# httpsworldview/openmeters

Measured on AMD Instinct MI355X. Metric: STFT frames/s (4096-pt Hann, hop 256, reassignment on), higher is better.
Workload: dtype f32

## Files before the change

openmeters_amd/csrc/buffer_device.hpp:

```cpp
#pragma once
#include <hip/hip_runtime.h>

#include "fft_device.hpp"

namespace omx {

struct GlobalBuffer {
    __amdgpu_buffer_rsrc_t rsrc;
};
__device__ __forceinline__ GlobalBuffer global_buffer(const void* base, uint32_t bytes) {
#ifdef OMX_BUFFER_NO_PIN
    return GlobalBuffer{__builtin_amdgcn_make_buffer_rsrc(const_cast<void*>(base), 0, (int)bytes, 0x00020000)};
#endif
    const uint64_t p = reinterpret_cast<uint64_t>(base);
    const uint32_t lo = (uint32_t)__builtin_amdgcn_readfirstlane((int)(uint32_t)p), hi = (uint32_t)__builtin_amdgcn_readfirstlane((int)(uint32_t)(p >> 32));
    const void* ub = reinterpret_cast<const void*>(((uint64_t)hi << 32) | lo);
    return GlobalBuffer{__builtin_amdgcn_make_buffer_rsrc(const_cast<void*>(ub), 0, __builtin_amdgcn_readfirstlane((int)bytes), 0x00020000)};
}
__device__ __forceinline__ float load_f32(const GlobalBuffer& b, uint32_t lane_bytes, uint32_t uniform_bytes) {
    return __builtin_bit_cast(float, __builtin_amdgcn_raw_buffer_load_b32(b.rsrc, (int)lane_bytes, (int)uniform_bytes, 0));
}
__device__ __forceinline__ v2f load_v2f(const GlobalBuffer& b, uint32_t lane_bytes, uint32_t uniform_bytes) {
    typedef unsigned u2 __attribute__((ext_vector_type(2)));
    const u2 u = __builtin_amdgcn_raw_buffer_load_b64(b.rsrc, (int)lane_bytes, (int)uniform_bytes, 0);
    return __builtin_bit_cast(v2f, u);
}

}
```

openmeters_amd/csrc/capi.cpp:

```cpp
#include "common.hpp"
#include "spectrogram.hpp"
#include "spectrum.hpp"
#include "loudness.hpp"
#include "stereometer.hpp"
#include "capture_group.hpp"
#include "oscilloscope.hpp"
#include "waveform.hpp"

namespace omx {
const std::string& last_error();
}
using namespace omx;

#define REQUIRE_DEVICE()                       \
    do {                                       \
        const int _rc = device_ready();        \
        if (_rc != OMX_NONE) return _rc;       \
    } while (0)

struct omx_spectrogram {
    SpectrogramSingle impl;
    explicit omx_spectrogram(const omx_spectrogram_config& c) : impl(c) {}
};
struct omx_spectrogram_bank {
// ... 228 lines not shown
    k_weighting_transition_debug(sample_rate, frames, out);
    return OMX_NONE;
}
int omx_debug_k2_phase_cycles(uint64_t* out, uint32_t n, int reset) {
    if (!out || n < (uint32_t)K2_PHASES) return OMX_ERR_INVALID;
    REQUIRE_DEVICE();
#ifndef OMX_TUNING
    (void)reset;
    set_last_error("omx_debug_k2_phase_cycles: phase-timing kernels exist only in the tuning build (make TUNING=1)");
    return OMX_ERR_UNSUPPORTED;
#else
    return guarded([&] {
        unsigned long long c[K2_PHASES];
        k2_phase_cycles(c, reset != 0);
        for (int i = 0; i < K2_PHASES; ++i) out[i] = c[i];
        return (int)K2_PHASES;
    });
#endif
}
int omx_spectrogram_bank_process_ragged(omx_spectrogram_bank* b, const float* pcm, uint64_t frames_capacity, const uint32_t* frames,
                                        const uint8_t* reset_mask, uint32_t channels, float sample_rate,
                                        const uint8_t positions[OMX_MAX_CHANNELS], void* stream, omx_spectrogram_ragged_update* out) {
    if (!b || !pcm || !frames || !positions) return OMX_ERR_INVALID;
    return guarded([&] {
        return b->impl.process_ragged(pcm, frames_capacity, frames, reset_mask, channels, sample_rate, positions, static_cast<hipStream_t>(stream), out);
    });
}
int omx_spectrogram_bank_set_option(omx_spectrogram_bank* b, uint32_t option, uint64_t value) {
    if (!b) return OMX_ERR_INVALID;
    switch (option) {
        case OMX_OPT_KERNEL_TIMING: b->impl.timer().enabled = value != 0; return OMX_NONE;
        case OMX_OPT_FORCE_GENERIC: b->impl.force_generic(value != 0); return OMX_NONE;
        case OMX_OPT_KERNEL_FORM:
            if (value != 0 && value != 1 && value != 2 && value != 30 && value != 31) return OMX_ERR_INVALID;
#ifndef OMX_TUNING
            if (value == 1 || value == 2) {
                set_last_error("OMX_OPT_KERNEL_FORM 1 / 2: superseded kernels, built by `make TUNING=1` (libomx_hip_tuning.so) only");
                return OMX_ERR_UNSUPPORTED;
            }
#endif
            b->impl.kernel_form((int)value);
            return OMX_NONE;
        default: return OMX_ERR_INVALID;
    }
}

void omx_spectrum_config_default(omx_spectrum_config* out) {
    if (out) spectrum_config_default(out);
}
int omx_spectrum_create(const omx_spectrum_config* cfg, omx_spectrum** out) {
    if (!cfg || !out) return OMX_ERR_INVALID;
    REQUIRE_DEVICE();
    return guarded([&] {
        *out = new omx_spectrum(*cfg);
        return (int)OMX_NONE;
    });
}
void omx_spectrum_destroy(omx_spectrum* h) { delete h; }
int omx_spectrum_get_config(const omx_spectrum* h, omx_spectrum_config* out) {
    if (!h || !out) return OMX_ERR_INVALID;
    *out = h->impl.bank.config();
    return OMX_NONE;
}
int omx_spectrum_update_config(omx_spectrum* h, const omx_spectrum_config* cfg) {
    if (!h || !cfg) return OMX_ERR_INVALID;
    return guarded([&] {
        h->impl.bank.update_config(*cfg, nullptr);
        return (int)OMX_NONE;
    });
}
// ... 632 lines not shown
```

openmeters_amd/csrc/spectrogram.cpp:

```cpp
#include "spectrogram.hpp"

namespace omx {

constexpr size_t kDefaultFftSize = 2048;
constexpr size_t kDefaultHopSize = 64;
constexpr size_t kMaxHistoryColumns = 8192;
constexpr size_t kHistoryByteBudget = 128u * 1024u * 1024u;

void spectrogram_config_default(omx_spectrogram_config* c) {
    std::memset(c, 0, sizeof(*c));
    c->sample_rate = kDefaultSampleRate;
    c->window = OMX_WINDOW_HANN;
    c->fft_size = kDefaultFftSize;
    c->hop_size = kDefaultHopSize;
    c->history_length = 0;
    c->zero_padding_factor = 1;
    c->use_reassignment = 1;
}

static void normalize(omx_spectrogram_config& c) {
    c.sample_rate = sanitize_sample_rate(c.sample_rate);
    if (c.fft_size == 0) c.fft_size = kDefaultFftSize;
    if (c.hop_size == 0) c.hop_size = std::max<uint64_t>(std::min<uint64_t>(kDefaultHopSize, c.fft_size), 1);
    c.zero_padding_factor = std::max<uint64_t>(c.zero_padding_factor, 1);
// ... 121 lines not shown
            OMX_HIP(hipStreamSynchronize(stream));
        }
        std::vector<float> tw(W);
        const float center = (float)(W ? W - 1 : 0) * 0.5f;
        for (size_t i = 0; i < W; ++i) tw[i] = ((float)i - center) * window[i];
        d_twindow_.upload(tw, stream);
        double sum = 0.0, squares = 0.0;
        for (float xf : window) {
            const double x = (double)xf;
            sum = sum + x;
            squares = squares + x * x;
        }
        power_scale_ = (float)(sum * sum / ((double)fft_size_ * squares));
    } else {
        power_scale_ = 1.0f;
    }
    fast4096_ = (W == fft_size_ && (W == 16384 || W == 8192 || W == 4096 || W == 2048 || W == 1024));
    const bool fast_classic_zp = !reassign && W < fft_size_ && W >= 256 &&
                                 (fft_size_ == 1024 || fft_size_ == 2048 || fft_size_ == 4096 || fft_size_ == 8192 || fft_size_ == 16384);
    fast_zp_ = reassign && W < fft_size_ &&
               (((W == 1024 || W == 2048 || W == 4096) && (fft_size_ == 2048 || fft_size_ == 4096 || fft_size_ == 8192)) ||
                ((W == 1024 || W == 2048 || W == 4096 || W == 8192) && fft_size_ == 16384));
    const bool residue_shape = W < fft_size_ && fft_size_ > 16384 && fft_size_ <= (size_t(1) << 19) && (fft_size_ & (fft_size_ - 1)) == 0 &&
                               (W == 1024 || W == 2048 || W == 4096 || W == 8192 || W == 16384);
    fast_zpr_ = reassign && residue_shape;
    classic_zpr_ = !reassign && residue_shape;
    if (fast_zpr_ || classic_zpr_) fast_zp_ = true;
    if (fast_classic_zp) {
        fast4096_ = true;
        d_tw256_.upload(twiddle_table(256, 256), stream);
        d_tw4096_.upload(twiddle_table(fft_size_, fft_size_), stream);
    } else if (fast4096_ || fast_zp_) {
        d_tw256_.upload(twiddle_table(256, 256), stream);
        d_tw4096_.upload(twiddle_table(W, W), stream);
        std::vector<float> half_tw = twiddle_table(2 * W, W);
        for (float& x : half_tw) x *= 0.5f;
        d_tw8192_.upload(half_tw, stream);
        if (fast_zp_) d_twF_.upload(twiddle_table(fft_size_, fft_size_), stream);
    }
    d_bin_norm_.upload(bin_norm, stream);
    OMX_HIP(hipStreamSynchronize(stream));
    prepared_ = true;

    const uint64_t buffered_len = (uint64_t)active_len * 2;
    const uint64_t pending = head_ - tail_;
    drain(pending > buffered_len ? pending - buffered_len : 0);
    pending_skip_ = 0;
}

void SpectrogramBank::prepare(hipStream_t stream) {
    if (!prepared_) rebuild_fft(stream);
}

void SpectrogramBank::update_config(const omx_spectrogram_config& in, hipStream_t stream) {
    omx_spectrogram_config cfg = in;
    normalize(cfg);
    const omx_spectrogram_config prev = cfg_;
    const bool prepared = prepared_;
    if (prepared) require_supported(cfg);
    const uint64_t old_read_len = prev.use_reassignment ? hilbert_len_ : prev.fft_size;
    cfg_ = cfg;
    const bool rate_changed = prev.sample_rate != cfg.sample_rate;
    const bool rebuild = prev.fft_size != cfg.fft_size || prev.zero_padding_factor != cfg.zero_padding_factor ||
                         prev.window != cfg.window || prev.use_reassignment != cfg.use_reassignment || rate_changed;
    if (rebuild && prepared) {
        rebuild_fft(stream);
        if (rate_changed) {
// ... 28 lines not shown
    if (cols) OMX_HIP(hipMemsetAsync(d_counts_.ptr, 0, (size_t)(n_streams_ * n_cols) * sizeof(uint32_t), stream));
    if (reassign) d_points_.reserve((size_t)(n_streams_ * n_cols * stride), pinned);
    else d_codes_.reserve((size_t)(n_streams_ * n_cols * stride), pinned);

    const float sr = cfg_.sample_rate;
    const float bin_hz = sr / (float)fft_size_;
    const float max_hz = sr * 0.5f;
    const float inv_2pi = sr / kTau;
    const float inv_hop = 1.0f / (float)hop;
    const float latency_hops = (float)center_offset * inv_hop;

    timer_.begin(stream);
    const bool fast = (fast4096_ || fast_zp_) && !force_generic_ && ring_cap_ <= (uint64_t(1) << 30) && hop <= 0xFFFFFFFFull;
    if (fast) {
        StftFastArgs fa{};
        fa.ring = ring_.ptr;
        fa.cap = ring_cap_;
        fa.tail = tail;
        fa.tails = tails;
        fa.cols = cols;
        fa.hop = (uint32_t)hop;
        fa.n_streams = n_streams_;
        fa.n_cols = (uint32_t)n_cols;
        fa.column_stride = (uint32_t)stride;
        fa.window_size = (uint32_t)W;
        fa.last_nonzero = last_nonzero_.ptr;
        fa.window = d_window_.ptr;
        fa.dwindow = d_dwindow_.ptr;
        fa.twindow = d_twindow_.ptr;
        fa.bin_norm = d_bin_norm_.ptr;
        fa.tw256 = reinterpret_cast<const v2f*>(d_tw256_.ptr);
        fa.tw4096 = reinterpret_cast<const v2f*>(d_tw4096_.ptr);
        fa.tw8192 = reinterpret_cast<const v2f*>(d_tw8192_.ptr);
        fa.bin_hz = bin_hz;
        fa.max_hz = max_hz;
        fa.inv_2pi = inv_2pi;
        fa.inv_hop = inv_hop;
        fa.latency_hops = latency_hops;
        fa.win_terms = (cfg_.window == OMX_WINDOW_HANN || cfg_.window == OMX_WINDOW_HAMMING) ? 2u : 0u;
        fa.win_c0 = cfg_.window == OMX_WINDOW_HANN ? 0.5f : 25.0f / 46.0f;
        fa.win_c1 = cfg_.window == OMX_WINDOW_HANN ? -0.5f : -21.0f / 46.0f;
        {
            static const float kCos[5][4] = {{1.0f, 0.0f, 0.0f, 0.0f},
                                             {0.5f, -0.5f, 0.0f, 0.0f},
                                             {25.0f / 46.0f, -21.0f / 46.0f, 0.0f, 0.0f},
                                             {0.42f, -0.5f, 0.08f, 0.0f},
                                             {0.35875f, -0.48829f, 0.14128f, -0.01168f}};
            static const uint32_t kTerms[5] = {1, 2, 2, 3, 4};
            const uint32_t wk = cfg_.window <= OMX_WINDOW_BLACKMAN_HARRIS ? cfg_.window : OMX_WINDOW_HANN;
            for (int m = 0; m < 4; ++m) fa.cos_c[m] = kCos[wk][m];
            fa.cos_terms = kTerms[wk];
        }
        fa.points = d_points_.ptr;
        fa.counts = d_counts_.ptr;
        if (!reassign) {
            d_col_sums_.reserve((size_t)(n_streams_ * n_cols));
            fa.col_sums = d_col_sums_.ptr;
        }
        const bool cross_check = kernel_form_ == 30;
        const bool split_check = kernel_form_ == 31;
        if (reassign && fft_size_ == 4096 && !fast_zp_ && split_check) {
            const uint64_t total = (uint64_t)n_streams_ * n_cols, chunk = std::min<uint64_t>(total, 4096);
            d_workspace_.reserve((size_t)(chunk * stft_big_scratch_bytes_per_frame() / sizeof(float)));
            for (uint64_t first = 0; first < total; first += chunk)
                launch_stft_reassigned_4096_split(fa, d_workspace_.ptr, (uint32_t)first, (uint32_t)std::min(chunk, total - first), stream);
        } else if (reassign && fft_size_ == 16384 && !fast_zp_) {
            const uint64_t total = (uint64_t)n_streams_ * n_cols, chunk = std::min<uint64_t>(total, 1024);
            d_workspace_.reserve((size_t)(chunk * stft_big_scratch_bytes_per_frame() / sizeof(float)));
            for (uint64_t first = 0; first < total; first += chunk)
                launch_stft_reassigned_16384(fa, d_workspace_.ptr, (uint32_t)first, (uint32_t)std::min(chunk, total - first), stream);
        } else if (fast_zpr_) {
            const uint64_t total = (uint64_t)n_streams_ * n_cols, per = stft_residue_scratch_bytes_per_frame((uint32_t)W, (uint32_t)fft_size_);
            const uint64_t chunk = std::min<uint64_t>(total, std::max<uint64_t>((uint64_t(512) << 20) / per, 1));
            d_workspace_.reserve((size_t)(chunk * per / sizeof(float)));
            for (uint64_t first = 0; first < total; first += chunk)
                (void)launch_stft_reassigned_residue(fa, (uint32_t)W, (uint32_t)(fft_size_ / W), reinterpret_cast<const v2f*>(d_twF_.ptr), d_workspace_.ptr,
                                                     (uint32_t)first, (uint32_t)std::min(chunk, total - first), stream);
        } else if (classic_zpr_) {
            (void)launch_stft_classic_residue(fa, d_codes_.ptr, (uint32_t)W, (uint32_t)(fft_size_ / W), reinterpret_cast<const v2f*>(d_twF_.ptr), stream);
        } else if (fast_zp_ && fft_size_ == 16384) {
            const uint64_t total = (uint64_t)n_streams_ * n_cols, chunk = std::min<uint64_t>(total, 1024);
            d_workspace_.reserve((size_t)(chunk * stft_big_scratch_bytes_per_frame() / sizeof(float)));
            for (uint64_t first = 0; first < total; first += chunk)
                (void)launch_stft_reassigned_zp_16384(fa, (uint32_t)W, reinterpret_cast<const v2f*>(d_twF_.ptr), d_workspace_.ptr,
                                                      (uint32_t)first, (uint32_t)std::min(chunk, total - first), stream);
        } else if (fast_zp_)
            (void)launch_stft_reassigned_zp(fa, (uint32_t)W, (uint32_t)fft_size_, reinterpret_cast<const v2f*>(d_twF_.ptr), stream);
// ... 390 lines not shown
```

openmeters_amd/csrc/spectrogram.hpp:

```cpp
#pragma once
#include "stft_kernels.hpp"

namespace omx {

void spectrogram_config_default(omx_spectrogram_config* c);
uint64_t col_byte_stride(uint32_t kind, uint32_t points);
uint64_t history_columns(uint32_t kind, uint32_t points, uint64_t requested);
uint16_t pack_classic_db_host(float db);

class SpectrogramBank {
public:
    SpectrogramBank(const omx_spectrogram_config& cfg, uint32_t n_streams);
    const omx_spectrogram_config& config() const { return cfg_; }
    void update_config(const omx_spectrogram_config& cfg, hipStream_t stream);
    void reset_audio();
    void prepare(hipStream_t stream);
    int process(const float* pcm, bool pcm_on_device, uint64_t frames, uint32_t channels, float sample_rate,
                const uint8_t positions[OMX_MAX_CHANNELS], hipStream_t stream, omx_spectrogram_bank_update* out);
    int push_begin(uint64_t frames, uint32_t channels, float sample_rate, hipStream_t stream, IngestSlots& slots);
    void push_end(const IngestSlots& slots);
    int process_pushed(hipStream_t stream, omx_spectrogram_bank_update* out);
    int process_ragged(const float* d_pcm, uint64_t frames_capacity, const uint32_t* frames, const uint8_t* reset_mask, uint32_t channels,
                       float sample_rate, const uint8_t positions[OMX_MAX_CHANNELS], hipStream_t stream, omx_spectrogram_ragged_update* out);
    int ragged_plan(const float* d_pcm, uint64_t frames_capacity, const uint32_t* frames, const uint8_t* reset_mask, uint32_t channels,
                    float sample_rate, const uint8_t positions[OMX_MAX_CHANNELS], hipStream_t stream, IngestArgs& ia_out);
    int ragged_finish(hipStream_t stream, omx_spectrogram_ragged_update* out);
    int fetch_column(uint64_t stream_index, uint64_t column, void* dst, uint64_t cap, uint64_t* n_out, hipStream_t stream);
    EventTimer& timer() { return timer_; }
    void force_generic(bool on) { force_generic_ = on; }
    void kernel_form(int form) { kernel_form_ = form; }
    void host_outputs(size_t limit_bytes) { host_output_limit_ = limit_bytes; }
    bool outputs_on_host() const { return d_counts_.pinned; }
    hipStream_t last_stream() const { return last_stream_; }

private:
    void rebuild_fft(hipStream_t stream);
    void launch_columns(uint64_t n_cols, uint64_t tail, const uint64_t* tails, const uint32_t* cols, hipStream_t stream);
    void enter_ragged(hipStream_t stream);
    void ensure_ring(uint64_t incoming, hipStream_t stream);
    void drain(uint64_t count);
    void advance(uint64_t count);
    void clear_last_nonzero(hipStream_t stream);

    omx_spectrogram_config cfg_{};
    uint32_t n_streams_;
    int kernel_form_ = 0;
    bool prepared_ = false, reset_ = true, fast4096_ = false, fast_zp_ = false, fast_zpr_ = false, classic_zpr_ = false, force_generic_ = false;
    size_t fft_size_ = 0, hilbert_len_ = 0;
    float power_scale_ = 1.0f;
    uint64_t head_ = 0, tail_ = 0, pending_skip_ = 0, ring_cap_ = 0;
    DeviceBuffer<float> ring_;
    HostStage staging_;
    DeviceBuffer<long long> last_nonzero_, partial_nonzero_;
    DeviceBuffer<float> d_window_, d_dwindow_, d_twindow_, d_bin_norm_, d_col_sums_;
    DeviceBuffer<float> d_tw_fft_, d_tw_hilbert_, d_tw256_, d_tw4096_, d_tw8192_, d_twF_, d_workspace_;
    DeviceBuffer<float> d_blu_chirp_, d_blu_bf_, d_blu_tw_;
    size_t blu_m_ = 0;
    OutBuffer<omx_spectrogram_point> d_points_;
    OutBuffer<uint32_t> d_counts_;
    OutBuffer<uint16_t> d_codes_;
    size_t host_output_limit_ = 0;
    uint64_t pend_max_cols_ = 0;
    bool ragged_ = false;
    uint64_t ragged_pending_bound_ = 0;
    DeviceBuffer<uint64_t> r_head_, r_tail_, r_skip_, r_ing_head_, r_col_tail_;
    DeviceBuffer<uint32_t> r_reset_flag_, r_ing_skip_, r_ing_count_, r_ncols_, r_reset_out_;
    DeviceView<uint32_t> r_frames_;
    DeviceView<uint8_t> r_mask_;
    RaggedStaging r_staging_;
    uint64_t last_cols_ = 0, last_stride_ = 0;
    uint32_t last_kind_ = OMX_COLUMN_REASSIGNED;
    EventTimer timer_;
    hipStream_t last_stream_ = nullptr;
};

struct SpectrogramSingle {
    SpectrogramBank bank;
    std::vector<uint64_t> offsets;
    std::vector<omx_spectrogram_point> points;
    std::vector<uint16_t> codes;
    explicit SpectrogramSingle(const omx_spectrogram_config& c) : bank(c, 1) { bank.host_outputs(size_t(2) << 20); }
    int process_block(const omx_block* block, omx_spectrogram_update* out);
};

}
```

openmeters_amd/csrc/stft4096_tri_kernels.hip:

```cpp
#include "stft_kernels.hpp"

#include <mutex>

#include "buffer_device.hpp"
#include "fft_device.hpp"
#include "fft_fused_device.hpp"
#include "reassign_device.hpp"
#include "twiddle_run_device.hpp"

namespace omx {

namespace {

#if !defined(TRI_KNOCK) || !defined(OMX_TUNING)
#undef TRI_KNOCK
#define TRI_KNOCK 0
#endif
#ifndef TRI_LDS_SYNC
#define TRI_LDS_SYNC 1
#endif
#if TRI_KNOCK == 3
#define TRI_SYNC() __builtin_amdgcn_sched_barrier(0)
#elif TRI_LDS_SYNC
#define TRI_SYNC() asm volatile("s_waitcnt lgkmcnt(0)\n\ts_barrier" ::: "memory")
#else
#define TRI_SYNC() __syncthreads()
#endif

__device__ __forceinline__ bool tri_block_to_stream_chunk(uint32_t n_streams, uint32_t chunks, uint32_t& s, uint32_t& chunk) {
    const uint32_t b = blockIdx.x;
    const uint32_t xcd = b & 7u, q = b >> 3;
    s = (q / chunks) * 8u + xcd;
    chunk = q % chunks;
    return s < n_streams;
}

template <int TT>
__device__ __forceinline__ v2f w8_at(v2f base) {
    return rotate128<4 * TT>(base);
}

#ifndef TRI_SWZ
#define TRI_SWZ 0
#endif
#if TRI_SWZ
constexpr int kTriSlots = 4096;
__device__ __forceinline__ int xslot(int j) { return j ^ ((j >> 4) & 15); }
__device__ __forceinline__ int per_call(int x) {
    asm volatile("" : "+v"(x));
// ... 88 lines not shown
#pragma unroll
    for (int t = 1; t < 16; ++t) w[t] = tw2[k * (unsigned)t];
    w[0] = w[1];
    dft16_fused_tw<INV>(v, w);
#else
#pragma unroll
    for (int t = 1; t < 16; ++t) v[t] = twmul<INV>(v[t], tw2[k * (unsigned)t]);
    dft16<INV>(v);
#endif
}
template <bool INV>
__device__ __forceinline__ void pass3_16(v2f (&v)[16], const v2f (&tw3)[15]) {
    if (TRI_KNOCK == 2) return;
#if TRI_FUSED
    v2f w[16];
#pragma unroll
    for (int t = 1; t < 16; ++t) w[t] = tw3[t - 1];
    w[0] = w[1];
    dft16_fused_tw<INV>(v, w);
#else
#pragma unroll
    for (int t = 1; t < 16; ++t) v[t] = twmul<INV>(v[t], tw3[t - 1]);
    dft16<INV>(v);
#endif
}
__device__ __forceinline__ void natural(v2f (&v)[16]) {
    v2f r[16];
#pragma unroll
    for (int t = 0; t < 16; ++t) r[t] = v[DFT16_OUT(t)];
#pragma unroll
    for (int t = 0; t < 16; ++t) v[t] = r[t];
}

template <bool INV>
__device__ __forceinline__ void tri_dual(v2f (&a)[16], v2f (&b)[16], v2f* X, const v2f* tw2, const v2f (&tw3)[15], int j) {
    plain16<INV>(a);
    x_write1(a, X, j);
    TRI_SYNC();
    x_read2(a, X, j);
    plain16<INV>(b);
    TRI_SYNC();
    x_write1(b, X, j);
    pass2_16<INV>(a, tw2, j);
    TRI_SYNC();
    x_read2(b, X, j);
    TRI_SYNC();
    x_write2(a, X, j);
    pass2_16<INV>(b, tw2, j);
    TRI_SYNC();
    x_read(a, X, j);
    TRI_SYNC();
    x_write2(b, X, j);
    pass3_16<INV>(a, tw3);
    natural(a);
    TRI_SYNC();
    x_read(b, X, j);
    pass3_16<INV>(b, tw3);
    natural(b);
}

__device__ __forceinline__ void store_point(omx_spectrogram_point* out, uint32_t pos, const omx_spectrogram_point& p) {
    *reinterpret_cast<omx_spectrogram_point*>(reinterpret_cast<char*>(out) + __umul24(pos, 12u)) = p;
}

}

constexpr size_t kTriLds = (size_t)kTriSlots * sizeof(v2f) + 4096 * sizeof(float) + 256 * sizeof(v2f) + 36 * sizeof(uint32_t) + 4 * sizeof(float);

template <int TERMS>
__global__ __launch_bounds__(256, 3) void stft_reassigned_4096_tri_kernel(StftFastArgs a) {
    extern __shared__ __attribute__((aligned(16))) unsigned char smem_raw[];
    v2f* X = reinterpret_cast<v2f*>(smem_raw);
    float* imb = reinterpret_cast<float*>(X + kTriSlots);
    v2f* tw2_lds = reinterpret_cast<v2f*>(imb + 4096);
    uint32_t* scan = reinterpret_cast<uint32_t*>(tw2_lds + 256);
    float* hil = reinterpret_cast<float*>(scan + 36);

    const uint32_t chunks = (a.n_cols + 1u) / 2u;
    uint32_t s, chunk;
    if (!tri_block_to_stream_chunk(a.n_streams, chunks, s, chunk)) return;
    const int j = threadIdx.x;
    const unsigned ju = threadIdx.x;
    const int lane = j & 63, wave = j >> 6;
    const int wave_u = __builtin_amdgcn_readfirstlane(wave);
    const float* ring = a.ring + (uint64_t)s * a.cap;
    const uint32_t mask32 = (uint32_t)(a.cap - 1);
    const uint32_t bytemask = mask32 << 2;
    const char* ring_bytes = reinterpret_cast<const char*>(ring);
    const long long last_nonzero = a.last_nonzero[s];
    const uint32_t* cols_p = a.cols;
    const uint64_t* tails_p = a.tails;
    const uint32_t n_cols_s = cols_p ? cols_p[s] : a.n_cols;
    const uint64_t tail_s = tails_p ? tails_p[s] : a.tail;
    const ReassignConsts rc{a.bin_hz, a.max_hz, a.inv_2pi, a.inv_hop, a.latency_hops};

    const uint32_t col0 = chunk * 2u;
    if (col0 >= n_cols_s) return;
    const bool have1 = col0 + 1u < n_cols_s;
    const uint32_t col1 = have1 ? col0 + 1u : col0;
    const uint64_t p0a = tail_s + (uint64_t)col0 * a.hop, p0b = tail_s + (uint64_t)col1 * a.hop;
    uint32_t* count_a = a.counts + (uint64_t)s * a.n_cols + col0;
    uint32_t* count_b = a.counts + (uint64_t)s * a.n_cols + col1;

    const uint32_t pa32 = (uint32_t)p0a, pb32 = (uint32_t)p0b;
    const uint32_t off_a = pa32 & mask32, hop_bytes = (pb32 - pa32) * 4u;
    const bool direct = (uint64_t)off_a + (uint64_t)(pb32 - pa32) + 8192ull <= a.cap && ((p0a | p0b) & 1ull) == 0;
    const GlobalBuffer windowb = global_buffer(ring + off_a, hop_bytes + 8192u * 4u);
    const GlobalBuffer tw4096b = global_buffer(a.tw4096, 4096u * 8u), tw8192b = global_buffer(a.tw8192, 4096u * 8u),
                       normb = global_buffer(a.bin_norm, 2049u * 4u), twinb = global_buffer(a.twindow, 4096u * 4u);

    v2f va[16], vb[16];
    if (TRI_KNOCK == 7) {
#pragma unroll
        for (int t = 0; t < 16; ++t) {
            va[t] = v2f{(float)(j + t) * 1e-4f, (float)(j - t) * 1e-4f};
            vb[t] = v2f{(float)(j + 2 * t) * 1e-4f, (float)(j - 3 * t) * 1e-4f};
        }
    } else if (direct) {
#pragma unroll
        for (int t = 0; t < 16; ++t) {
            va[t] = load_v2f(windowb, ju * 8u, 2048u * (unsigned)t);
            vb[t] = load_v2f(windowb, ju * 8u, hop_bytes + 2048u * (unsigned)t);
        }
    } else {
#pragma unroll
        for (int t = 0; t < 16; ++t) {
            const uint32_t qa = pa32 + 2u * (ju + 256u * (unsigned)t), qb = pb32 + 2u * (ju + 256u * (unsigned)t);
            va[t] = v2f{ring[qa & mask32], ring[(qa + 1u) & mask32]};
            vb[t] = v2f{ring[qb & mask32], ring[(qb + 1u) & mask32]};
        }
    }
    v2f tw3[15];
#pragma unroll
    for (int t = 1; t < 16; ++t) tw3[t - 1] = load_v2f(tw4096b, ju * 8u * (unsigned)t, 0);
    tw2_lds[j] = a.tw256[ju];
    const v2f w8_base = load_v2f(tw8192b, ju * 8u, 0);
    const bool silent_a = last_nonzero < (long long)p0a, silent_b = last_nonzero < (long long)p0b;
    if (silent_a && (silent_b || !have1)) {
        if (j == 0) {
            *count_a = 0;
            if (have1) *count_b = 0;
        }
        return;
    }
    tri_dual<false>(va, vb, X, tw2_lds, tw3, j);

    const int part = j ? xslot(256 - j) : kTriStep;
    auto hilbert_spectrum = [&](v2f (&y)[16], const v2f (&v)[16]) {
#pragma unroll
        for (int t = 0; t < 16; ++t) {
            const v2f z = v[t], zr = TRI_KNOCK == 8 ? v[15 - t] : X[part + kTriStep * (15 - t)];
            const v2f sum{z.x + zr.x, z.y - zr.y}, dif{z.x - zr.x, z.y + zr.y};
            v2f w8;
            switch (t) {
                case 0: w8 = w8_at<0>(w8_base); break;
                case 1: w8 = w8_at<1>(w8_base); break;
                case 2: w8 = w8_at<2>(w8_base); break;
                case 3: w8 = w8_at<3>(w8_base); break;
                case 4: w8 = w8_at<4>(w8_base); break;
                case 5: w8 = w8_at<5>(w8_base); break;
                case 6: w8 = w8_at<6>(w8_base); break;
                case 7: w8 = w8_at<7>(w8_base); break;
                case 8: w8 = w8_at<8>(w8_base); break;
                case 9: w8 = w8_at<9>(w8_base); break;
                case 10: w8 = w8_at<10>(w8_base); break;
                case 11: w8 = w8_at<11>(w8_base); break;
                case 12: w8 = w8_at<12>(w8_base); break;
                case 13: w8 = w8_at<13>(w8_base); break;
                case 14: w8 = w8_at<14>(w8_base); break;
                default: w8 = w8_at<15>(w8_base); break;
            }
            y[t] = TRI_KNOCK == 5 ? sum + dif : cmulc(sum, w8) - cmul(dif, w8);
            if (t == 0 && j == 0) y[t] = v2f{0.0f, 0.0f};
        }
    };
    v2f ya[16], yb[16];
    TRI_SYNC();
#pragma unroll
    for (int t = 0; t < 16; ++t) X[xslot(j) + kTriStep * t] = va[t];
    if (j == 0) {
        hil[0] = (va[0].x + va[0].y) * 0.5f;
// ... 22 lines not shown
            for (int t = 0; t < 16; ++t) xr[t] = *reinterpret_cast<const float*>(ring_bytes + (((q + 256u * (unsigned)t) << 2) & bytemask));
        }
    };
    auto load_twindow = [&](float (&twin)[16]) {
#pragma unroll
        for (int t = 0; t < 16; ++t) twin[t] = load_f32(twinb, ju * 4u, 1024u * (unsigned)t);
    };
    float xra[16], twina[16];
    load_real_half(xra, 0u, pa32);
    load_twindow(twina);
    TRI_SYNC();
    float* imag_a = reinterpret_cast<float*>(X);
#pragma unroll
    for (int t = 4; t < 12; ++t) {
        *reinterpret_cast<v2f*>(imag_a + 2 * (j + 256 * t - 1024)) = ya[t];
        *reinterpret_cast<v2f*>(imb + 2 * (j + 256 * t - 1024)) = yb[t];
    }
    TRI_SYNC();
    constexpr int REACH = TERMS > 1 ? TERMS - 1 : 1;
    const float c0 = a.cos_c[0];
    float half_c[REACH], dscale[REACH];
#pragma unroll
    for (int m = 1; m <= REACH; ++m) {
        half_c[m - 1] = TERMS > 1 ? 0.5f * a.cos_c[m] : 0.0f;
        dscale[m - 1] = TERMS > 1 ? a.cos_c[m] * ((float)m * 3.14159265358979323846f / 4096.0f) : 0.0f;
    }
    v2f* lin_z = X;

    struct ColumnPoints {
        omx_spectrogram_point pts[9];
        unsigned long long masks[9];
        uint32_t exc, running;
    };
    auto build = [&](v2f (&z)[16], v2f (&z2)[16], const float (&xr)[16], const float (&twin)[16], const float* imag, float half_x0, float half_xn) {
        const float par = (j & 1) ? -half_xn : half_xn;
#pragma unroll
        for (int t = 0; t < 16; ++t) {
            z[t] = v2f{4096.0f * xr[t] - half_x0 + par, imag[j + 256 * t]};
            z2[t] = v2f{z[t].x * twin[t], z[t].y * twin[t]};
        }
    };
    auto analyse = [&](v2f (&z)[16], v2f (&z2)[16], bool silent, ColumnPoints& o) {
        omx_spectrogram_point (&pts)[9] = o.pts;
        unsigned long long (&masks)[9] = o.masks;
        TRI_SYNC();
        tri_dual<false>(z, z2, X, tw2_lds, tw3, j);
        float pn[9];
#pragma unroll
        for (int t = 0; t < 9; ++t) pn[t] = load_f32(normb, ju * 4u, 1024u * (unsigned)t);
        TRI_SYNC();
#pragma unroll
        for (int t = 0; t < 8; ++t) lin_z[3 + j + 256 * t] = z[t];
        if (wave_u == 0) lin_z[3 + j + 2048] = z[8];
        if (j >= 253) lin_z[j - 253] = z[15];
        TRI_SYNC();
        auto bins = [&](auto first, auto last) {
            constexpr int T0 = decltype(first)::value, T1 = decltype(last)::value;
            v2f nzm[T1 - T0][REACH], nzp[T1 - T0][REACH];
            if constexpr (TERMS > 1) {
#pragma unroll
                for (int t = T0; t < T1; ++t)
#pragma unroll
                    for (int m = 1; m <= REACH; ++m) {
                        nzm[t - T0][m - 1] = lin_z[3 + j + 256 * t - m];
                        nzp[t - T0][m - 1] = lin_z[3 + j + 256 * t + m];
                    }
            }
#pragma unroll
            for (int t = T0; t < T1; ++t) {
                const uint32_t bin = (uint32_t)(j + 256 * t);
                v2f bb{c0 * z[t].x, c0 * z[t].y}, bd{0.0f, 0.0f};
// ... 33 lines not shown
            bins(std::integral_constant<int, 2>{}, std::integral_constant<int, 3>{});
            bins(std::integral_constant<int, 3>{}, std::integral_constant<int, 4>{});
            bins(std::integral_constant<int, 4>{}, std::integral_constant<int, 5>{});
            bins(std::integral_constant<int, 5>{}, std::integral_constant<int, 6>{});
            bins(std::integral_constant<int, 6>{}, std::integral_constant<int, 7>{});
            bins(std::integral_constant<int, 7>{}, std::integral_constant<int, 8>{});
        }
        if (wave_u == 0) {
            bins(std::integral_constant<int, 8>{}, std::integral_constant<int, 9>{});
        } else {
            masks[8] = 0ull;
            if (lane == 0) scan[32 + wave] = 0u;
        }
        TRI_SYNC();
        const uint32_t cnt = lane < 36 ? scan[lane] : 0u;
        const uint32_t inc = wave_inclusive_sum(cnt);
        o.exc = inc - cnt;
        o.running = (uint32_t)__builtin_amdgcn_readlane((int)inc, 35);
    };
    auto store = [&](const ColumnPoints& o, uint32_t col, uint32_t* count_out) {
        omx_spectrogram_point* out = a.points + ((uint64_t)s * a.n_cols + col) * a.column_stride;
#pragma unroll
        for (int t = 0; t < 9; ++t) {
            const uint32_t before = (uint32_t)__builtin_amdgcn_readlane((int)o.exc, 4 * t + wave_u);
            if (TRI_KNOCK != 4 && ((o.masks[t] >> lane) & 1ull)) {
                const uint32_t pos = before + lanes_below(o.masks[t]);
                store_point(out, pos, o.pts[t]);
            }
        }
        if (j == 0) *count_out = o.running;
    };
    v2f z[16], z2[16];
    ColumnPoints pts;
    build(z, z2, xra, twina, imag_a, half_x0a, half_xna);
    analyse(z, z2, silent_a, pts);
    store(pts, col0, count_a);
    if (have1) {
        float xrb[16], twinb_v[16];
        load_real_half(xrb, hop_bytes, pb32);
        load_twindow(twinb_v);
        build(z, z2, xrb, twinb_v, imb, half_x0b, half_xnb);
        analyse(z, z2, silent_b, pts);
        store(pts, col1, count_b);
    }
}

template <int TERMS>
static void launch_tri(const StftFastArgs& a, hipStream_t stream) {
    static std::once_flag attr_once;
    std::call_once(attr_once, [] {
        (void)hipFuncSetAttribute(reinterpret_cast<const void*>(stft_reassigned_4096_tri_kernel<TERMS>), hipFuncAttributeMaxDynamicSharedMemorySize,
                                  (int)kTriLds);
    });
    const uint32_t chunks = (a.n_cols + 1u) / 2u;
    hipLaunchKernelGGL(stft_reassigned_4096_tri_kernel<TERMS>, dim3(stream_column_grid(a.n_streams, chunks)), dim3(256), kTriLds, stream, a);
}

void launch_stft_reassigned_4096_tri(const StftFastArgs& a, hipStream_t stream) {
    if (a.n_cols == 0 || a.n_streams == 0) return;
    switch (a.cos_terms) {
        case 1: launch_tri<1>(a, stream); break;
        case 2: launch_tri<2>(a, stream); break;
        case 3: launch_tri<3>(a, stream); break;
        default: launch_tri<4>(a, stream); break;
    }
}

}
```

openmeters_amd/csrc/stft_kernels.hip:

```cpp
#include "stft_kernels.hpp"

#include "fft_device.hpp"
#ifdef OMX_TUNING
#include "fft_wave_device.hpp"
#endif

namespace omx {

__device__ __forceinline__ float project_lr(int channel, float left, float right) {
    switch (channel) {
        case OMX_CHANNEL_LEFT: return left;
        case OMX_CHANNEL_RIGHT: return right;
        case OMX_CHANNEL_MID: return (left + right) * 0.5f;
        case OMX_CHANNEL_SIDE: return (left - right) * 0.5f;
        default: return 0.0f;
    }
}

constexpr int INGEST_FRAMES_PER_THREAD = 16;
constexpr int INGEST_FRAMES_PER_WG = 256 * INGEST_FRAMES_PER_THREAD;

__global__ __launch_bounds__(256) void ingest_project_kernel(IngestArgs a) {
    __shared__ long long wave_best[4];
    const uint32_t s = blockIdx.y;
// ... 1041 lines not shown
    OMX_HIP(hipMemcpyFromSymbol(out, HIP_SYMBOL(g_k2_phase_cycles), K2_PHASES * sizeof(unsigned long long)));
    if (reset) {
        const unsigned long long zero[K2_PHASES] = {};
        OMX_HIP(hipMemcpyToSymbol(HIP_SYMBOL(g_k2_phase_cycles), zero, sizeof(zero)));
    }
}

using K2Default = K2Variant<1, true, true, true, true, false, 2, false, true, false, true>;
#endif

int stft_reassigned_4096_transforms_per_frame() { return 4; }

void launch_stft_reassigned_4096(const StftFastArgs& a, int form, hipStream_t stream) {
    if (a.n_cols == 0 || a.n_streams == 0) return;
#ifndef OMX_TUNING
    (void)form;
    launch_stft_reassigned_4096_tri(a, stream);
#else
    if (form == 0 && a.win_terms == 2) {
        static const int swz_variant = [] {
            const char* e = getenv("OMX_K2_VARIANT");
            return e ? atoi(e) : 0;
        }();
        if (swz_variant == 50) { launch_stft_reassigned_4096_swz_pair(a, stream); return; }
        if (swz_variant == 51) { launch_stft_reassigned_4096_col(a, stream); return; }
    }
    {
        static const int env_form = [] {
            const char* e = tuning_env("OMX_K2_FORM");
            return e ? atoi(e) : -1;
        }();
        const int f = (form == 0 && env_form >= 0) ? env_form : form;
        if (f == 0 && a.cos_terms >= 1 && a.cos_terms <= 4) { launch_stft_reassigned_4096_tri(a, stream); return; }
        if (f == 2 && a.win_terms == 2) { launch_stft_reassigned_4096_pair(a, stream); return; }
    }
    static const int variant = [] {
        const char* e = getenv("OMX_K2_VARIANT");
        return e ? atoi(e) : 0;
    }();
    switch (variant) {
        case 100: launch_k2_variant<K2Variant<1, false, false, true, false>>(a, stream); return;
        case 1: launch_k2_variant<K2Variant<1, false, false, true, true>>(a, stream); return;
        case 2: launch_k2_variant<K2Variant<1, true, false, true, false>>(a, stream); return;
        case 3: launch_k2_variant<K2Variant<1, false, true, true, false>>(a, stream); return;
        case 13: launch_k2_variant<K2Variant<1, true, true, false, false, true, 3, true>>(a, stream); return;
        case 20: launch_k2_wave(a, stream); return;
        case 9: launch_k2_variant<K2Variant<1, true, true, true, true, false, 2, false, true, true, true>>(a, stream); return;
        case 41: launch_k2_variant<K2Variant<1, true, true, true, true, false, 2, false, true, false, true, false, false, 1>>(a, stream); return;
        case 42: launch_k2_variant<K2Variant<1, true, true, true, true, false, 2, false, true, false, true, false, false, 2>>(a, stream); return;
        case 43: launch_k2_variant<K2Variant<1, true, true, true, true, false, 2, false, true, false, true, false, false, 3>>(a, stream); return;
        case 44: launch_k2_variant<K2Variant<1, true, true, true, true, false, 2, false, true, false, true, false, false, 4>>(a, stream); return;
        case 45: launch_k2_variant<K2Variant<1, true, true, true, true, false, 2, false, true, false, true, false, false, 5>>(a, stream); return;
        case 47: launch_k2_variant<K2Variant<1, true, true, true, true, false, 2, false, true, false, true, false, false, 7>>(a, stream); return;
        case 48: launch_k2_variant<K2Variant<1, true, true, true, true, false, 2, false, true, false, true, false, false, 8>>(a, stream); return;
        case 49: launch_k2_variant<K2Variant<1, true, true, true, true, false, 2, false, true, false, true, false, false, 9>>(a, stream); return;
        case 46: launch_k2_variant<K2Variant<1, true, true, true, true, false, 2, false, true, false, true, false, false, 6>>(a, stream); return;
        case 14: launch_k2_variant<K2Variant<1, true, true, true, true, false, 2, false, true, false, true, false, true>>(a, stream); return;
        case 8: launch_k2_variant<K2Variant<1, true, true, true, true, false, 2, false, true, true, true, true>>(a, stream); return;
        case 7: launch_k2_variant<K2Variant<1, true, true, true, true, false, 2, false, true, true, false>>(a, stream); return;
        case 12: launch_k2_variant<K2Variant<1, true, true, true, true>>(a, stream); return;
        default: break;
    }
    launch_k2_variant<K2Default>(a, stream);
#endif
}

// ... 138 lines not shown
```

openmeters_amd/csrc/stft_kernels.hpp:

```cpp
#pragma once
#include "bluestein_plan.hpp"
#include "common.hpp"

namespace omx {

typedef float v2f __attribute__((ext_vector_type(2)));

constexpr int OMX_INGEST_MAX_OUT = 3;
constexpr int OMX_PROJECT_RAW = -1;

struct IngestArgs {
    const float* pcm;
    uint64_t frames_total;
    uint64_t skip;
    uint64_t count;
    AudioFormatArgs fmt;
    int n_out;
    int project[OMX_INGEST_MAX_OUT];
    float* ring[OMX_INGEST_MAX_OUT];
    uint64_t cap;
    uint64_t head;
    long long* last_nonzero;
    long long* partial_nonzero;
    const uint32_t* skips;
// ... 68 lines not shown
    uint64_t head;
    uint64_t n_windows;
    uint32_t hop, window;
    uint32_t slots, slot0;
    uint32_t first_hop, n_hops;
    uint32_t n_streams;
    float* carry;
    float* sums;
    const uint64_t* tails;
    const uint64_t* froms;
    const uint64_t* heads;
    const uint32_t* slot0s;
    const uint32_t* modes;
};
void launch_window_sums_carry(const WindowCarryArgs& a, hipStream_t stream);

struct StftFastArgs {
    const float* ring;
    uint64_t cap;
    uint64_t tail;
    uint32_t hop;
    uint32_t n_streams;
    uint32_t n_cols;
    uint32_t column_stride;
    uint32_t window_size;
    const long long* last_nonzero;
    const float* window;
    const float* dwindow;
    const float* twindow;
    const float* bin_norm;
    const v2f* tw256;
    const v2f* tw4096;
    const v2f* tw8192;
    float bin_hz, max_hz, inv_2pi, inv_hop, latency_hops;
    float win_c0, win_c1;
    uint32_t win_terms;
    float cos_c[4];
    uint32_t cos_terms;
    const uint64_t* tails;
    const uint32_t* cols;
    omx_spectrogram_point* points;
    uint32_t* counts;
    float* col_sums;
};
__device__ __forceinline__ uint64_t stft_tail(const StftFastArgs& a, uint32_t s) { return a.tails ? a.tails[s] : a.tail; }
__device__ __forceinline__ uint32_t stft_cols(const StftFastArgs& a, uint32_t s) { return a.cols ? a.cols[s] : a.n_cols; }
constexpr int K2_PHASES = 12;
void k2_phase_cycles(unsigned long long out[K2_PHASES], bool reset);
unsigned long long* k2_phase_buffer();
void launch_stft_reassigned_4096(const StftFastArgs& a, int form, hipStream_t stream);
int stft_reassigned_4096_transforms_per_frame();
void launch_stft_reassigned_4096_pair(const StftFastArgs& a, hipStream_t stream);
void launch_stft_reassigned_4096_tri(const StftFastArgs& a, hipStream_t stream);
void launch_stft_reassigned_4096_swz_pair(const StftFastArgs& a, hipStream_t stream);
void launch_stft_reassigned_4096_col(const StftFastArgs& a, hipStream_t stream);
uint32_t stream_column_grid(uint32_t n_streams, uint32_t n_cols);
void launch_stft_reassigned_pow2(const StftFastArgs& a, uint32_t fft_size, hipStream_t stream);
void launch_stft_reassigned_8192(const StftFastArgs& a, hipStream_t stream);
constexpr int kBigHalo = 16;
template <int LOGN>
constexpr int kBigRow = (1 << LOGN) / 2 + 1 + 2 * kBigHalo;
struct BigScratch {
    v2f* sv;
    v2f* spec;
    uint32_t first;
    uint32_t count;
};
uint64_t stft_residue_scratch_bytes_per_frame(uint32_t window, uint32_t fft_size);
bool launch_stft_classic_residue(const StftFastArgs& a, uint16_t* codes, uint32_t window, uint32_t zp, const v2f* twF, hipStream_t stream);
bool launch_stft_reassigned_residue(const StftFastArgs& a, uint32_t window, uint32_t zp, const v2f* twF, void* scratch, uint32_t first, uint32_t count,
                                    hipStream_t stream);
void launch_hilbert_16k(const StftFastArgs& a, const BigScratch& sc, bool imag_only, hipStream_t stream);
void launch_windowed_reassign_16k(const StftFastArgs& a, const BigScratch& sc, bool imag_only, hipStream_t stream);
void launch_windowed_16k(const StftFastArgs& a, const BigScratch& sc, hipStream_t stream);
uint64_t stft_big_scratch_bytes_per_frame();
void launch_stft_reassigned_16384(const StftFastArgs& a, void* scratch, uint32_t first, uint32_t count, hipStream_t stream);
bool launch_stft_reassigned_zp_16384(const StftFastArgs& a, uint32_t window, const v2f* twF, void* scratch, uint32_t first, uint32_t count,
                                     hipStream_t stream);
void launch_stft_reassigned_4096_split(const StftFastArgs& a, void* scratch, uint32_t first, uint32_t count, hipStream_t stream);
bool launch_stft_reassigned_zp(const StftFastArgs& a, uint32_t window, uint32_t fft_size, const v2f* twF, hipStream_t stream);
void launch_stft_classic_pow2(const StftFastArgs& a, uint16_t* codes, uint32_t fft_size, hipStream_t stream);

struct StftGenericArgs {
    const float* ring;
    uint64_t cap;
    uint64_t tail;
// ... 107 lines not shown
```

Before: 37.80 million.

## Raise tri STFT kernel to four workgroups per CU by parking imaginary slice globally

Shrinks the tri 4096 reassigned kernel's LDS so four workgroups fit per CU. The separate imaginary buffer is dropped by overlaying it on the transform slots, and the second frame's imaginary half is parked in a global scratch buffer. Stage-3 twiddles are preloaded as a transposed table and reloaded after the sync instead of living in registers. The aim is more occupancy. The cost is extra global traffic for the parked data, twiddle reloads, and a new scratch allocation. The old 3-per-CU path is kept as form 3 for tuning builds only.

Measured after the change: 36.43 million. -3.6%, worse.

```diff
diff --git a/openmeters_amd/csrc/buffer_device.hpp b/openmeters_amd/csrc/buffer_device.hpp
--- a/openmeters_amd/csrc/buffer_device.hpp
+++ b/openmeters_amd/csrc/buffer_device.hpp
@@ -25,5 +25,8 @@
     const u2 u = __builtin_amdgcn_raw_buffer_load_b64(b.rsrc, (int)lane_bytes, (int)uniform_bytes, 0);
     return __builtin_bit_cast(v2f, u);
 }
+__device__ __forceinline__ void store_f32(const GlobalBuffer& b, float v, uint32_t lane_bytes, uint32_t uniform_bytes) {
+    __builtin_amdgcn_raw_buffer_store_b32(__builtin_bit_cast(unsigned, v), b.rsrc, (int)lane_bytes, (int)uniform_bytes, 0);
+}
 
 }
diff --git a/openmeters_amd/csrc/capi.cpp b/openmeters_amd/csrc/capi.cpp
--- a/openmeters_amd/csrc/capi.cpp
+++ b/openmeters_amd/csrc/capi.cpp
@@ -284,10 +284,10 @@
         case OMX_OPT_KERNEL_TIMING: b->impl.timer().enabled = value != 0; return OMX_NONE;
         case OMX_OPT_FORCE_GENERIC: b->impl.force_generic(value != 0); return OMX_NONE;
         case OMX_OPT_KERNEL_FORM:
-            if (value != 0 && value != 1 && value != 2 && value != 30 && value != 31) return OMX_ERR_INVALID;
+            if (value != 0 && value != 1 && value != 2 && value != 3 && value != 30 && value != 31) return OMX_ERR_INVALID;
 #ifndef OMX_TUNING
-            if (value == 1 || value == 2) {
-                set_last_error("OMX_OPT_KERNEL_FORM 1 / 2: superseded kernels, built by `make TUNING=1` (libomx_hip_tuning.so) only");
+            if (value == 1 || value == 2 || value == 3) {
+                set_last_error("OMX_OPT_KERNEL_FORM 1 / 2 / 3: superseded kernels, built by `make TUNING=1` (libomx_hip_tuning.so) only");
                 return OMX_ERR_UNSUPPORTED;
             }
 #endif
diff --git a/openmeters_amd/csrc/spectrogram.cpp b/openmeters_amd/csrc/spectrogram.cpp
--- a/openmeters_amd/csrc/spectrogram.cpp
+++ b/openmeters_amd/csrc/spectrogram.cpp
@@ -177,7 +177,17 @@
         d_tw4096_.upload(twiddle_table(fft_size_, fft_size_), stream);
     } else if (fast4096_ || fast_zp_) {
         d_tw256_.upload(twiddle_table(256, 256), stream);
-        d_tw4096_.upload(twiddle_table(W, W), stream);
+        const std::vector<float> tw_w = twiddle_table(W, W);
+        d_tw4096_.upload(tw_w, stream);
+        if (reassign && W == 4096 && fast4096_) {
+            std::vector<float> tw3t(15 * 256 * 2);
+            for (size_t t = 1; t < 16; ++t)
+                for (size_t j = 0; j < 256; ++j) {
+                    tw3t[((t - 1) * 256 + j) * 2] = tw_w[j * t * 2];
+                    tw3t[((t - 1) * 256 + j) * 2 + 1] = tw_w[j * t * 2 + 1];
+                }
+            d_tw3t_.upload(tw3t, stream);
+        }
         std::vector<float> half_tw = twiddle_table(2 * W, W);
         for (float& x : half_tw) x *= 0.5f;
         d_tw8192_.upload(half_tw, stream);
@@ -272,6 +282,7 @@
         fa.tw256 = reinterpret_cast<const v2f*>(d_tw256_.ptr);
         fa.tw4096 = reinterpret_cast<const v2f*>(d_tw4096_.ptr);
         fa.tw8192 = reinterpret_cast<const v2f*>(d_tw8192_.ptr);
+        fa.tw3t = reinterpret_cast<const v2f*>(d_tw3t_.ptr);
         fa.bin_hz = bin_hz;
         fa.max_hz = max_hz;
         fa.inv_2pi = inv_2pi;
@@ -293,6 +304,10 @@
         }
         fa.points = d_points_.ptr;
         fa.counts = d_counts_.ptr;
+        if (reassign && fft_size_ == 4096 && !fast_zp_ && d_points_.pinned) {
+            d_park_.reserve((size_t)(n_streams_ * ((n_cols + 1) / 2) * 4096));
+            fa.park = d_park_.ptr;
+        }
         if (!reassign) {
             d_col_sums_.reserve((size_t)(n_streams_ * n_cols));
             fa.col_sums = d_col_sums_.ptr;
diff --git a/openmeters_amd/csrc/spectrogram.hpp b/openmeters_amd/csrc/spectrogram.hpp
--- a/openmeters_amd/csrc/spectrogram.hpp
+++ b/openmeters_amd/csrc/spectrogram.hpp
@@ -54,6 +54,7 @@
     DeviceBuffer<long long> last_nonzero_, partial_nonzero_;
     DeviceBuffer<float> d_window_, d_dwindow_, d_twindow_, d_bin_norm_, d_col_sums_;
     DeviceBuffer<float> d_tw_fft_, d_tw_hilbert_, d_tw256_, d_tw4096_, d_tw8192_, d_twF_, d_workspace_;
+    DeviceBuffer<float> d_tw3t_, d_park_;
     DeviceBuffer<float> d_blu_chirp_, d_blu_bf_, d_blu_tw_;
     size_t blu_m_ = 0;
     OutBuffer<omx_spectrogram_point> d_points_;
diff --git a/openmeters_amd/csrc/stft4096_tri_kernels.hip b/openmeters_amd/csrc/stft4096_tri_kernels.hip
--- a/openmeters_amd/csrc/stft4096_tri_kernels.hip
+++ b/openmeters_amd/csrc/stft4096_tri_kernels.hip
@@ -15,6 +15,16 @@
 #if !defined(TRI_KNOCK) || !defined(OMX_TUNING)
 #undef TRI_KNOCK
 #define TRI_KNOCK 0
+#endif
+#ifndef TRI_WG_PER_CU
+#define TRI_WG_PER_CU 4
+#endif
+#if TRI_WG_PER_CU != 3 && TRI_WG_PER_CU != 4
+#error "TRI_WG_PER_CU is 3 or 4"
+#endif
+#if TRI_WG_PER_CU == 3
+#define stft_reassigned_4096_tri_kernel stft_reassigned_4096_tri3_kernel
+#define launch_stft_reassigned_4096_tri launch_stft_reassigned_4096_tri3
 #endif
 #ifndef TRI_LDS_SYNC
 #define TRI_LDS_SYNC 1
@@ -169,8 +179,19 @@
     for (int t = 0; t < 16; ++t) v[t] = r[t];
 }
 
+#if TRI_WG_PER_CU == 4
+typedef GlobalBuffer Tw3Source;
+__device__ __forceinline__ void load_tw3(v2f (&tw3)[15], const GlobalBuffer& tw3tb, int j) {
+    uint32_t lane_bytes = (uint32_t)j * 8u;
+    asm volatile("" : "+v"(lane_bytes));
+#pragma unroll
+    for (int t = 0; t < 15; ++t) tw3[t] = load_v2f(tw3tb, lane_bytes, 2048u * (unsigned)t);
+}
+#else
+typedef v2f Tw3Source[15];
+#endif
 template <bool INV>
-__device__ __forceinline__ void tri_dual(v2f (&a)[16], v2f (&b)[16], v2f* X, const v2f* tw2, const v2f (&tw3)[15], int j) {
+__device__ __forceinline__ void tri_dual(v2f (&a)[16], v2f (&b)[16], v2f* X, const v2f* tw2, const Tw3Source& tw3_source, int j) {
     plain16<INV>(a);
     x_write1(a, X, j);
     TRI_SYNC();
@@ -185,6 +206,12 @@
     x_write2(a, X, j);
     pass2_16<INV>(b, tw2, j);
     TRI_SYNC();
+#if TRI_WG_PER_CU == 4
+    v2f tw3[15];
+    load_tw3(tw3, tw3_source, j);
+#else
+    const v2f (&tw3)[15] = tw3_source;
+#endif
     x_read(a, X, j);
     TRI_SYNC();
     x_write2(b, X, j);
@@ -202,14 +229,21 @@
 
 }
 
-constexpr size_t kTriLds = (size_t)kTriSlots * sizeof(v2f) + 4096 * sizeof(float) + 256 * sizeof(v2f) + 36 * sizeof(uint32_t) + 4 * sizeof(float);
+constexpr int kTriImbFloats = TRI_WG_PER_CU == 3 ? 4096 : 0;
+constexpr size_t kTriLds = (size_t)kTriSlots * sizeof(v2f) + kTriImbFloats * sizeof(float) + 256 * sizeof(v2f) + 36 * sizeof(uint32_t) + 4 * sizeof(float);
+static_assert(TRI_WG_PER_CU == 3 || (kTriLds <= 160 * 1024 / 4 && (size_t)kTriSlots * sizeof(v2f) >= 2 * 4096 * sizeof(float)),
+              "four workgroups per CU: 40 KiB of LDS each, and both imaginary half-slices cross the transform buffer at once");
 
 template <int TERMS>
-__global__ __launch_bounds__(256, 3) void stft_reassigned_4096_tri_kernel(StftFastArgs a) {
+__global__ __launch_bounds__(256, (TRI_WG_PER_CU == 4 && TERMS <= 2) ? 4 : 3) void stft_reassigned_4096_tri_kernel(StftFastArgs a) {
     extern __shared__ __attribute__((aligned(16))) unsigned char smem_raw[];
     v2f* X = reinterpret_cast<v2f*>(smem_raw);
+#if TRI_WG_PER_CU == 4
+    float* imb = reinterpret_cast<float*>(X) + 4096;
+#else
     float* imb = reinterpret_cast<float*>(X + kTriSlots);
-    v2f* tw2_lds = reinterpret_cast<v2f*>(imb + 4096);
+#endif
+    v2f* tw2_lds = reinterpret_cast<v2f*>(reinterpret_cast<float*>(X + kTriSlots) + kTriImbFloats);
     uint32_t* scan = reinterpret_cast<uint32_t*>(tw2_lds + 256);
     float* hil = reinterpret_cast<float*>(scan + 36);
 
@@ -243,7 +277,7 @@
     const uint32_t off_a = pa32 & mask32, hop_bytes = (pb32 - pa32) * 4u;
     const bool direct = (uint64_t)off_a + (uint64_t)(pb32 - pa32) + 8192ull <= a.cap && ((p0a | p0b) & 1ull) == 0;
     const GlobalBuffer windowb = global_buffer(ring + off_a, hop_bytes + 8192u * 4u);
-    const GlobalBuffer tw4096b = global_buffer(a.tw4096, 4096u * 8u), tw8192b = global_buffer(a.tw8192, 4096u * 8u),
+    const GlobalBuffer tw8192b = global_buffer(a.tw8192, 4096u * 8u),
                        normb = global_buffer(a.bin_norm, 2049u * 4u), twinb = global_buffer(a.twindow, 4096u * 4u);
 
     v2f va[16], vb[16];
@@ -267,11 +301,16 @@
             vb[t] = v2f{ring[qb & mask32], ring[(qb + 1u) & mask32]};
         }
     }
+#if TRI_WG_PER_CU == 4
+    const GlobalBuffer tw3 = global_buffer(a.tw3t, 15u * 256u * 8u);
+#else
+    const GlobalBuffer tw4096b = global_buffer(a.tw4096, 4096u * 8u);
     v2f tw3[15];
 #pragma unroll
     for (int t = 1; t < 16; ++t) tw3[t - 1] = load_v2f(tw4096b, ju * 8u * (unsigned)t, 0);
+#endif
     tw2_lds[j] = a.tw256[ju];
-    const v2f w8_base = load_v2f(tw8192b, ju * 8u, 0);
+    const v2f w8_entry = load_v2f(tw8192b, ju * 8u, 0);
     const bool silent_a = last_nonzero < (long long)p0a, silent_b = last_nonzero < (long long)p0b;
     if (silent_a && (silent_b || !have1)) {
         if (j == 0) {
@@ -284,6 +323,13 @@
 
     const int part = j ? xslot(256 - j) : kTriStep;
     auto hilbert_spectrum = [&](v2f (&y)[16], const v2f (&v)[16]) {
+#if TRI_WG_PER_CU == 4
+        float w8_re = w8_entry.x, w8_im = w8_entry.y;
+        asm volatile("" : "+v"(w8_re), "+v"(w8_im));
+        const v2f w8_base{w8_re, w8_im};
+#else
+        const v2f w8_base = w8_entry;
+#endif
 #pragma unroll
         for (int t = 0; t < 16; ++t) {
             const v2f z = v[t], zr = TRI_KNOCK == 8 ? v[15 - t] : X[part + kTriStep * (15 - t)];
@@ -372,11 +418,11 @@
         unsigned long long masks[9];
         uint32_t exc, running;
     };
-    auto build = [&](v2f (&z)[16], v2f (&z2)[16], const float (&xr)[16], const float (&twin)[16], const float* imag, float half_x0, float half_xn) {
+    auto build = [&](v2f (&z)[16], v2f (&z2)[16], const float (&xr)[16], const float (&twin)[16], auto imag, float half_x0, float half_xn) {
         const float par = (j & 1) ? -half_xn : half_xn;
 #pragma unroll
         for (int t = 0; t < 16; ++t) {
-            z[t] = v2f{4096.0f * xr[t] - half_x0 + par, imag[j + 256 * t]};
+            z[t] = v2f{4096.0f * xr[t] - half_x0 + par, imag(t)};
             z2[t] = v2f{z[t].x * twin[t], z[t].y * twin[t]};
         }
     };
@@ -476,14 +522,31 @@
     };
     v2f z[16], z2[16];
     ColumnPoints pts;
-    build(z, z2, xra, twina, imag_a, half_x0a, half_xna);
+#if TRI_WG_PER_CU == 4
+    const uint64_t park_wg = a.park ? (uint64_t)s * chunks + chunk : 0;
+    const void* park_base = a.park ? static_cast<const void*>(a.park + park_wg * 4096u)
+                                   : static_cast<const void*>(a.points + ((uint64_t)s * a.n_cols + col1) * a.column_stride);
+    const GlobalBuffer parkb = global_buffer(park_base, 4096u * 4u);
+    if (have1) {
+#pragma unroll
+        for (int t = 0; t < 16; ++t) store_f32(parkb, imb[j + 256 * t], ju * 4u, 1024u * (unsigned)t);
+    }
+#endif
+    build(z, z2, xra, twina, [&](int t) { return imag_a[j + 256 * t]; }, half_x0a, half_xna);
     analyse(z, z2, silent_a, pts);
     store(pts, col0, count_a);
     if (have1) {
         float xrb[16], twinb_v[16];
         load_real_half(xrb, hop_bytes, pb32);
         load_twindow(twinb_v);
-        build(z, z2, xrb, twinb_v, imb, half_x0b, half_xnb);
+#if TRI_WG_PER_CU == 4
+        float imb_v[16];
+#pragma unroll
+        for (int t = 0; t < 16; ++t) imb_v[t] = load_f32(parkb, ju * 4u, 1024u * (unsigned)t);
+        build(z, z2, xrb, twinb_v, [&](int t) { return imb_v[t]; }, half_x0b, half_xnb);
+#else
+        build(z, z2, xrb, twinb_v, [&](int t) { return imb[j + 256 * t]; }, half_x0b, half_xnb);
+#endif
         analyse(z, z2, silent_b, pts);
         store(pts, col1, count_b);
     }
diff --git a/openmeters_amd/csrc/stft_kernels.hip b/openmeters_amd/csrc/stft_kernels.hip
--- a/openmeters_amd/csrc/stft_kernels.hip
+++ b/openmeters_amd/csrc/stft_kernels.hip
@@ -1097,6 +1097,7 @@
         }();
         const int f = (form == 0 && env_form >= 0) ? env_form : form;
         if (f == 0 && a.cos_terms >= 1 && a.cos_terms <= 4) { launch_stft_reassigned_4096_tri(a, stream); return; }
+        if (f == 3 && a.cos_terms >= 1 && a.cos_terms <= 4) { launch_stft_reassigned_4096_tri3(a, stream); return; }
         if (f == 2 && a.win_terms == 2) { launch_stft_reassigned_4096_pair(a, stream); return; }
     }
     static const int variant = [] {
diff --git a/openmeters_amd/csrc/stft_kernels.hpp b/openmeters_amd/csrc/stft_kernels.hpp
--- a/openmeters_amd/csrc/stft_kernels.hpp
+++ b/openmeters_amd/csrc/stft_kernels.hpp
@@ -124,6 +124,7 @@
     const v2f* tw256;
     const v2f* tw4096;
     const v2f* tw8192;
+    const v2f* tw3t;
     float bin_hz, max_hz, inv_2pi, inv_hop, latency_hops;
     float win_c0, win_c1;
     uint32_t win_terms;
@@ -132,6 +133,7 @@
     const uint64_t* tails;
     const uint32_t* cols;
     omx_spectrogram_point* points;
+    float* park;
     uint32_t* counts;
     float* col_sums;
 };
@@ -144,6 +146,7 @@
 int stft_reassigned_4096_transforms_per_frame();
 void launch_stft_reassigned_4096_pair(const StftFastArgs& a, hipStream_t stream);
 void launch_stft_reassigned_4096_tri(const StftFastArgs& a, hipStream_t stream);
+void launch_stft_reassigned_4096_tri3(const StftFastArgs& a, hipStream_t stream);
 void launch_stft_reassigned_4096_swz_pair(const StftFastArgs& a, hipStream_t stream);
 void launch_stft_reassigned_4096_col(const StftFastArgs& a, hipStream_t stream);
 uint32_t stream_column_grid(uint32_t n_streams, uint32_t n_cols);
```
